# beecave-homelab/VibeVoice-ROCm

Measured on AMD Instinct MI355X. Metric: audio-sec/s, higher is better.
Workload: dtype bf16; 1 GPU; cfg2: VibeVoice-1.5B shapes, 1 speaker(s) x 203-frame voice prompt, 330-token prompt, 225 frames (30.0 s audio), CFG=2.0, 20 DPM-Solver++ steps, whole generate() incl. voice encode + prefill; global_batch=1, parallelism=replicas x1 (one dialogue per GPU), hipgraph=True

## Files before the change

### vibevoice_rocm_amd/build.py

```python
from __future__ import annotations

import hashlib
import os
import shutil
import subprocess
import sys

HERE = os.path.dirname(os.path.abspath(__file__))
ROOT = os.path.dirname(HERE)
SRC = [os.path.join(HERE, "csrc", f) for f in ("vv_kernels.hip", "vv_gemv_stream.hip", "vv_gemv_rows.hip", "vv_mfma_gemm.hip", "vv_block1d.hip", "vv_convffn.hip",
                                               "vv_fused.hip", "vv_attn_decode.hip", "vv_attn_prefill.hip", "vv_model.hip",
                                               "vv_nf4_import.hip")]
HDR = [os.path.join(ROOT, "include", "vv_hip.h"), os.path.join(HERE, "csrc", "vv_common.h")]
OUT = os.path.join(HERE, "libvv_hip.so")
OBJDIR = os.path.join(HERE, "csrc", "build")
STAMP = os.path.join(HERE, "libvv_hip.stamp")
FLAGS = ["--offload-arch=gfx950", "-O3", "-std=c++17", "-fPIC"]


def find_hipcc() -> str:
    for c in (os.environ.get("HIPCC"), shutil.which("hipcc"), "/opt/rocm/bin/hipcc"):
        if c and os.path.exists(c):
            return c
    raise RuntimeError("hipcc not found (ROCm toolchain required to build the MI355X kernels)")


def _flavour() -> str:
    return hashlib.sha256("\n".join([os.path.basename(s) for s in SRC] + FLAGS).encode()).hexdigest()[:16]


def _check_sources():
    missing = [p for p in SRC + HDR if not os.path.exists(p)]
    if missing:
        raise RuntimeError("missing kernel sources: " + ", ".join(os.path.relpath(p, ROOT) for p in missing))


def up_to_date() -> bool:
    if not os.path.exists(OUT):
        return False
    if not all(os.path.exists(p) for p in SRC + HDR):
        return True
    t = os.path.getmtime(OUT)
    if not all(os.path.getmtime(p) <= t for p in SRC + HDR):
        return False
    try:
        return open(STAMP).read().strip() == _flavour()
    except OSError:
        return False


def _obj(src: str) -> str:
    return os.path.join(OBJDIR, os.path.basename(src) + ".o")


def build(force: bool = False, verbose: bool = True, jobs: int = 6) -> str:
    if not force and up_to_date():
        return OUT
    _check_sources()
    os.makedirs(OBJDIR, exist_ok=True)
    flags = [*FLAGS, "-I" + os.path.join(ROOT, "include"), "-I" + os.path.join(HERE, "csrc")]
    hipcc = find_hipcc()
    hdr_t = max(os.path.getmtime(p) for p in HDR)
    todo = [s for s in SRC if force or not os.path.exists(_obj(s)) or os.path.getmtime(_obj(s)) < max(os.path.getmtime(s), hdr_t)]
    procs = []
    for s in todo:
        cmd = [hipcc, *flags, "-c", s, "-o", _obj(s)]
        if verbose:
            print(" ".join(cmd), flush=True)
        procs.append((s, subprocess.Popen(cmd)))
        while sum(p.poll() is None for _, p in procs) >= jobs:
            next(p for _, p in procs if p.poll() is None).wait()
    failed = [s for s, p in procs if p.wait() != 0]
    if failed:
        raise RuntimeError("hipcc failed for " + ", ".join(os.path.basename(f) for f in failed))
    cmd = [hipcc, "--offload-arch=gfx950", "-shared", "-fPIC", *[_obj(s) for s in SRC], "-o", OUT]
    if verbose:
        print(" ".join(cmd), flush=True)
    subprocess.run(cmd, check=True)
    with open(STAMP, "w") as f:
        f.write(_flavour() + "\n")
    return OUT


if __name__ == "__main__":
    build(force="--force" in sys.argv)
    print(OUT)
```

### vibevoice_rocm_amd/csrc/vv_common.h

```cpp
#ifndef VV_COMMON_H
#define VV_COMMON_H
#include <hip/hip_runtime.h>
#include <stdarg.h>
#include <stdint.h>
#include "vv_hip.h"

int vv_set_error(int code, const char* fmt, ...);

#define VV_CHECK_LAUNCH(name)                                                                    \
  do {                                                                                           \
    hipError_t e_ = hipGetLastError();                                                           \
    if (e_ != hipSuccess) return vv_set_error(VV_E_HIP, "%s: %s", name, hipGetErrorString(e_));  \
  } while (0)

#define VV_TRY(expr)            \
  do {                          \
    int rc_ = (expr);           \
    if (rc_) return rc_;        \
  } while (0)

int vv_launch_gemv_stream(const vv_lin_args& a, hipStream_t s);
int vv_launch_gemv_rows(const vv_lin_args& a, float* part, size_t part_floats, int* tickets, size_t n_tickets, hipStream_t s);
size_t vv_gemv_rows_part_floats(int n, int dual);
size_t vv_gemv_rows_tickets(int n);
int vv_gemv_rows_init();
void vv_gemv_rows_set(int on, int blocks, int pers);
int vv_linear_ws(const vv_lin_args* a, const void* f1, const void* f2, float* part, size_t part_floats, int* tickets, size_t n_tickets,
                 vv_stream_t stream, const vv_w8* q1 = nullptr, const vv_w8* q2 = nullptr);
int vv_launch_mfma_gemm(const vv_lin_args& a, hipStream_t s);
int vv_mfma_gemm_init();
int vv_launch_attn_decode(const float* qkv, int64_t ld_qkv, int R, int heads, const vv_kv* kv, int layer, const float2* rope, const int* lens, float* out,
                          int64_t ldo, float* part, int* tickets, int nsplit, int part_cap, hipStream_t s);
int vv_attn_decode_ws(const float* qkv, int64_t ld_qkv, int R, int heads, const vv_kv* kv, int layer, const float* rope_table, const int* lens, float* out,
                      int64_t ldo, float* part, int* tickets, int nsplit, int part_cap, vv_stream_t stream);
int vv_launch_attn_prefill(const float* qkv, int64_t ld_qkv, int R, int heads, const vv_kv* kv, int layer, const int* lens, const int* cache_rows,
                           float* out, int64_t ldo, hipStream_t s);
int vv_head_init_fused(const vv_head* h, const float* noise, float* Xs, float* Ms, float* h0, int64_t ldh, hipStream_t s);
bool vv_head_boundary_supported(const vv_head* h);
int vv_head_boundary_fused(const vv_head* h, const float* hrows, int64_t ldh, const float* shift, const float* scale, int64_t ld_mod, float cfg,
                           const vv_dpm_coef* k, float* Xs, float* Ms, float* h_out, int64_t ldh_out, float* latent_out, hipStream_t s);
int vv_head_boundary_batch(const vv_head* h, const float* hrows, int64_t ldh, const float* shift, const float* scale, int64_t ld_mod, float cfg,
                           const vv_dpm_coef* k, float* Xs, float* Ms, int64_t state_stride, float* h_out, int64_t ldh_out, float* latent_out,
                           int64_t latent_stride, int B, hipStream_t s,
                           const float* nx = nullptr, int64_t nx_stride = 0);
int vv_head_sde_proj_fused(const vv_head* h, const float* sde_noise, int64_t ld_sde, int n_steps, int B, float* NX, hipStream_t s);
int vv_fused_init();
int vv_head_pre_fused(const vv_head* h, const float* cond2, int64_t ld_cond, const float* temb, int n_steps, void* c_bf16, const float* noise,
                      float* Xs, float* Ms, float* h0, int64_t ldh, hipStream_t s);
int vv_launch_connector_pair(const vv_connector* ac, const vv_connector* sem, const float* latent, const float* semfeat, float* out, int64_t ldo, int rows_out,
                             float* ws, hipStream_t s);
int vv_head_modulations_fused(const vv_head* h, const void* c_bf16, int rows, float* const* mod, float* modf, hipStream_t s);
struct vv_conv_ctx_item { float* pad; float* state; int ctx, T, C; const float* dw_w; float* hs; int affine; float scale, bias; };
int vv_conv_ctx_batch(const vv_conv_ctx_item* items, int n, int scatter, hipStream_t s);
int vv_block1d_init();
int vv_launch_block1d(const vv_block& B, int wdt, const float* x, float* out, int T, int C, float eps, hipStream_t s);
void vv_block1d_set_fused(int on);
void vv_block1d_set_blocks(int b);
int vv_convffn_init();
int vv_launch_convffn(const vv_block& B, int wdt, const float* x, float* y, void* hidden, float* hist_new, float* out, int T, int C, float eps,
                      hipStream_t s);
void vv_convffn_set(int on);
int vv_launch_ffn_in_row(const vv_block& B, int wdt, const float* x, float* y, float* hidden, float* hist_new, int C, float eps, hipStream_t s);
void vv_convffn_set_t1(int on);
int vv_launch_ffn_in_row_hs(const vv_block& B, int wdt, const float* x, float* y, float* hidden, float* hist_new, int C, float eps, hipStream_t s);
void vv_convffn_set_t1hs(int on);
void vv_convffn_set_rows(int c, int rows);
void vv_convffn_set_c128(int on);
bool vv_convffn_prefers(int wdt, int T, int C);
int vv_launch_skinny(const vv_lin_args& a, hipStream_t s);
void vv_skinny_set(int on, int min_m, int max_m);
int vv_rmsnorm_rows(const float* x, int64_t ldx, const float* w, float eps, int rows, int n, float* out, int64_t ldo, hipStream_t s);

#ifdef __HIPCC__
__device__ __forceinline__ float vv_gelu_as(float v) {
  const float x = v * 0.70710678118654752440f, ax = fabsf(x);
  const float t = __builtin_amdgcn_rcpf(fmaf(0.3275911f, ax, 1.0f));
  const float poly = t * fmaf(t, fmaf(t, fmaf(t, fmaf(t, 1.061405429f, -1.453152027f), 1.421413741f), -0.284496736f), 0.254829592f);
  const float erf_abs = 1.0f - poly * __expf(-ax * ax);
  return 0.5f * v * (1.0f + copysignf(erf_abs, x));
}

__device__ __forceinline__ float vv_wave_sum(float v) {
#define VV_DPP_ADD(ctrl) v += __int_as_float(__builtin_amdgcn_update_dpp(0, __float_as_int(v), ctrl, 0xF, 0xF, true))
  VV_DPP_ADD(0xB1);
  VV_DPP_ADD(0x4E);
  VV_DPP_ADD(0x141);
  VV_DPP_ADD(0x140);
#undef VV_DPP_ADD
  const float r0 = __int_as_float(__builtin_amdgcn_readlane(__float_as_int(v), 0));
  const float r1 = __int_as_float(__builtin_amdgcn_readlane(__float_as_int(v), 16));
  const float r2 = __int_as_float(__builtin_amdgcn_readlane(__float_as_int(v), 32));
  const float r3 = __int_as_float(__builtin_amdgcn_readlane(__float_as_int(v), 48));
  return (r0 + r1) + (r2 + r3);
}
#endif

#endif
```

### vibevoice_rocm_amd/csrc/vv_gemv_stream.hip

```cpp
#include <hip/hip_runtime.h>
#include <stdint.h>

#include "vv_hip.h"
#include "vv_common.h"

namespace {

typedef unsigned short bf16_t;
typedef unsigned int u32x4 __attribute__((ext_vector_type(4)));

__device__ __forceinline__ float wsum(float v) { return vv_wave_sum(v); }
__device__ __forceinline__ float silu1(float v) { return v / (1.0f + expf(-v)); }
__device__ __forceinline__ float gelu1(float v) { return 0.5f * v * (1.0f + erff(v * 0.70710678118654752440f)); }

__device__ __forceinline__ void unpack8(const u32x4 v, float (&o)[8]) {
  o[0] = __uint_as_float(v.x << 16); o[1] = __uint_as_float(v.x & 0xffff0000u);
  o[2] = __uint_as_float(v.y << 16); o[3] = __uint_as_float(v.y & 0xffff0000u);
  o[4] = __uint_as_float(v.z << 16); o[5] = __uint_as_float(v.z & 0xffff0000u);
  o[6] = __uint_as_float(v.w << 16); o[7] = __uint_as_float(v.w & 0xffff0000u);
}

typedef unsigned int u32x2 __attribute__((ext_vector_type(2)));
typedef float f32x2 __attribute__((ext_vector_type(2)));
__device__ __forceinline__ void unpack8_f8(const u32x4 v, float (&o)[8]) {
// ... 450 lines not shown
    if (KSPLIT == 1) {
      if (lane < RW * M) {
        float v = acc[0][0], v2 = DUAL ? acc2[0][0] : 0.f;
#pragma unroll
        for (int r = 0; r < RW; ++r)
#pragma unroll
          for (int m = 0; m < M; ++m)
            if (lane == r * M + m) { v = acc[r][m]; if (DUAL) v2 = acc2[r][m]; }
        const int r = lane / M, m = lane - r * M;
        const int n = g * RW + r;
        if (n < N && m < mr) epi_pre(a, m, n, v, v2, eo_cur[0]);
      }
    } else {
      if (lane == 0) {
#pragma unroll
        for (int r = 0; r < RW; ++r)
#pragma unroll
          for (int m = 0; m < M; ++m) {
            part[parity][wave][(r * M + m) * 2] = acc[r][m];
            part[parity][wave][(r * M + m) * 2 + 1] = DUAL ? acc2[r][m] : 0.f;
          }
      }
      __syncthreads();
      if (tid < RW * M) {
        const int r = tid / M, m = tid - r * M;
        const int n = g * RW + r;
        if (n < N && m < mr) {
          float s = 0.f, s2 = 0.f;
#pragma unroll
          for (int w4 = 0; w4 < NW; ++w4) { s += part[parity][w4][tid * 2]; s2 += part[parity][w4][tid * 2 + 1]; }
          epi_pre(a, m, n, s, s2, eo_cur[0]);
        }
      }
      parity ^= 1;
    }
#pragma unroll
    for (int i = 0; i < NE; ++i) eo_cur[i] = eo_nxt[i];
#pragma unroll
    for (int r = 0; r < RW; ++r)
#pragma unroll
      for (int u = 0; u < KU; ++u) { cur[r][u] = nxt[r][u]; if (DUAL) cur2[r][u] = nxt2[r][u]; }
    g = gn;
    if (g + gstride < n_groups) { load_eo(eo_nxt, g + gstride); issue(nxt, nxt2, g + gstride); }
  }
}

int g_dual_rw = 1;

template <int M, bool DUAL, int KSPLIT, int KU, int RW>
void launch_rw(const vv_lin_args& a, hipStream_t s) {
  const int n_groups = (a.n + RW - 1) / RW;
  const int waves = (KSPLIT == 1 && g_waves_override >= 3 && g_waves_override <= 8) ? g_waves_override : 4;
  const int work = (KSPLIT == 1) ? (n_groups + waves - 1) / waves : n_groups;
  const int cap = (KSPLIT == 1) ? (DUAL ? (RW == 1 ? 512 : 448) : 512) : (a.k > 6144 ? g_long_cap : 1024);
  int blocks = work < cap ? work : cap;
  if (g_blocks_override > 0) blocks = g_blocks_override < work ? g_blocks_override : work;
  const int threads = KSPLIT == 1 ? 64 * waves : 64 * KSPLIT;
  if constexpr (RW == 4) {
    hipLaunchKernelGGL((gemv_stream_kernel<M, DUAL, KSPLIT, KU, RW, 2>), dim3(blocks), dim3(threads), 0, s, a, n_groups, g_opt);
    return;
  }
  if constexpr (M <= 2) {
    if (a.wdt == VV_FP8) {
      hipLaunchKernelGGL((gemv_stream_kernel<M, DUAL, KSPLIT, KU, RW, 1>), dim3(blocks), dim3(threads), 0, s, a, n_groups, g_opt);
      return;
    }
  }
  hipLaunchKernelGGL((gemv_stream_kernel<M, DUAL, KSPLIT, KU, RW, 0>), dim3(blocks), dim3(threads), 0, s, a, n_groups, g_opt);
}

int g_small_rw = 2;

template <int M, bool DUAL, int KSPLIT, int KU>
bool launch_one(const vv_lin_args& a, hipStream_t s) {
  if (a.wdt == VV_NF4) {
    if constexpr (M <= 2 && KSPLIT <= 8 && !(DUAL && KU > 4)) { launch_rw<M, DUAL, KSPLIT, KU, 4>(a, s); return true; }
    return false;
  }
  if (DUAL && g_dual_rw == 1) launch_rw<M, DUAL, KSPLIT, KU, 1>(a, s);
  else if (!DUAL && KSPLIT == 1 && a.n <= 4096 && g_small_rw == 1) launch_rw<M, DUAL, KSPLIT, KU, 1>(a, s);
  else launch_rw<M, DUAL, KSPLIT, KU, 2>(a, s);
  return true;
}

template <int M, bool DUAL, int KSPLIT>
bool launch_kus(const vv_lin_args& a, hipStream_t s, int ku) {
  switch (ku) {
    case 1: if constexpr (KSPLIT == 1) return launch_one<M, DUAL, KSPLIT, 1>(a, s); else return false;
    case 2: return launch_one<M, DUAL, KSPLIT, 2>(a, s);
    case 3: return launch_one<M, DUAL, KSPLIT, 3>(a, s);
    case 4: if constexpr (!DUAL || KSPLIT == 1) return launch_one<M, DUAL, KSPLIT, 4>(a, s); else return false;
    case 5: if constexpr (!DUAL || KSPLIT == 1) return launch_one<M, DUAL, KSPLIT, 5>(a, s); else return false;
  }
  return false;
}

template <int M, bool DUAL>
bool launch_ku(const vv_lin_args& a, hipStream_t s, int ksplit, int ku) {
  switch (ksplit) {
    case 1: return launch_kus<M, DUAL, 1>(a, s, ku);
    case 4: return launch_kus<M, DUAL, 4>(a, s, ku);
    case 8: return launch_kus<M, DUAL, 8>(a, s, ku);
    case 16: if constexpr (!DUAL) return launch_kus<M, false, 16>(a, s, ku); else return false;
  }
  return false;
}

bool launch_m8(const vv_lin_args& a, hipStream_t s, int ksplit, int ku) {
  if (ksplit == 1) {
    if (ku == 1) launch_rw<8, false, 1, 1, 1>(a, s); else launch_rw<8, false, 1, 2, 1>(a, s);
    return true;
  }
  switch (ksplit) {
    case 4: launch_rw<8, false, 4, 2, 2>(a, s); return true;
    case 8: launch_rw<8, false, 8, 2, 2>(a, s); return true;
  }
  return false;
}

}

void vv_gemv_stream_set_blocks(int b) { g_blocks_override = b; }
void vv_gemv_stream_set_waves(int w) { g_waves_override = w; }
void vv_gemv_stream_set_opt(int o) { g_opt = o; }
void vv_gemv_stream_set_long(int cap, int ku) { if (cap > 0) g_long_cap = cap; if (ku > 0) g_long_ku = ku; }
void vv_gemv_stream_set_dual_rw(int r) { g_dual_rw = r; }
void vv_gemv_stream_set_small_rw(int r) { g_small_rw = r; }

int vv_launch_gemv_stream(const vv_lin_args& a, hipStream_t s) {
  if ((a.wdt != VV_BF16 && a.wdt != VV_FP8 && a.wdt != VV_NF4) || a.m > 8 || a.k % 8) return 0;
  if (a.wdt == VV_NF4 && (a.m > 2 || a.k % 64 || !a.wscale || (a.w2 && !a.w2scale) || (uintptr_t)a.w % 16 || (a.w2 && (uintptr_t)a.w2 % 16) ||
                          (uintptr_t)a.wscale % 4 || (a.w2 && (uintptr_t)a.w2scale % 4) || (a.flags & VV_LIN_W_FRAG)))
    return 0;
  if (a.wdt == VV_FP8 && (a.m > 2 || !a.wscale || (a.w2 && !a.w2scale) || (uintptr_t)a.w % 8 || (a.w2 && (uintptr_t)a.w2 % 8))) return 0;
  if (a.m > 4) {
    if (a.w2 || a.wdt != VV_BF16) return 0;
    if ((uintptr_t)a.w % 16 || (uintptr_t)a.x % 16 || a.ldx % 4) return 0;
    if (a.norm_w && (uintptr_t)a.norm_w % 16) return 0;
    if (a.mod_scale && ((uintptr_t)a.mod_scale % 16 || (uintptr_t)a.mod_shift % 16 || a.ld_mod % 4)) return 0;
    const int units8 = (a.k + 511) / 512;
    int ks = 0, ku8 = 0;
    for (int w : {1, 4, 8}) {
      if ((units8 + w - 1) / w <= 2) { ks = w; ku8 = (units8 + w - 1) / w; break; }
    }
    if (!ks) return 0;
    if (ks > 1) ku8 = 2;
    return launch_m8(a, s, ks, ku8) ? 1 : 0;
  }
  if (a.wdt == VV_BF16 && ((uintptr_t)a.w % 16 || (a.w2 && (uintptr_t)a.w2 % 16))) return 0;
  if ((uintptr_t)a.x % 16) return 0;
  if (a.m > 1 && a.ldx % 4) return 0;
  if (a.norm_w && (uintptr_t)a.norm_w % 16) return 0;
  if (a.mod_scale && ((uintptr_t)a.mod_scale % 16 || (uintptr_t)a.mod_shift % 16 || a.ld_mod % 4)) return 0;
  const int units = (a.k + 511) / 512;
  const bool dual = a.w2 != nullptr;
  int ksplit = 1, ku = units;
  if (units > ((a.wdt == VV_NF4 && dual) ? 4 : 5)) {
    const int kumax = dual ? 3 : (units > 12 ? g_long_ku : 5);
    ksplit = 0;
    for (int w : {4, 8, 16}) {
      if ((units + w - 1) / w <= kumax) { ksplit = w; ku = (units + w - 1) / w; break; }
    }
    if (!ksplit) return 0;
    if (ku < 2) ku = 2;
  }
  if (a.wdt == VV_NF4 && ksplit > 8) return 0;
  bool ok;
  if (a.m == 1) ok = dual ? launch_ku<1, true>(a, s, ksplit, ku) : launch_ku<1, false>(a, s, ksplit, ku);
  else if (a.m == 2) ok = dual ? launch_ku<2, true>(a, s, ksplit, ku) : launch_ku<2, false>(a, s, ksplit, ku);
  else ok = dual ? launch_ku<4, true>(a, s, ksplit, ku) : launch_ku<4, false>(a, s, ksplit, ku);
  return ok ? 1 : 0;
}
```

### vibevoice_rocm_amd/csrc/vv_kernels.hip

```cpp
#include <hip/hip_runtime.h>
#include <hip/hip_bf16.h>
#include <stdint.h>
#include <stdio.h>
#include <string.h>
#include <math.h>

#include "vv_hip.h"
#include "vv_common.h"

static thread_local char g_err[512] = "";

int vv_set_error(int code, const char* fmt, ...) {
  va_list ap;
  va_start(ap, fmt);
  vsnprintf(g_err, sizeof(g_err), fmt, ap);
  va_end(ap);
  return code;
}

extern "C" const char* vv_last_error(void) { return g_err; }
extern "C" int vv_abi_version(void) { return 6; }
int vv_mixer_init();
extern "C" int vv_init(void) {
  VV_TRY(vv_mixer_init());
  VV_TRY(vv_mfma_gemm_init());
  VV_TRY(vv_block1d_init());
  VV_TRY(vv_convffn_init());
  VV_TRY(vv_gemv_rows_init());
  return vv_fused_init();
}
static float* g_rows_part = nullptr;
static int* g_rows_tk = nullptr;
static const size_t G_ROWS_PART_FLOATS = (size_t)4 << 20, G_ROWS_TICKETS = 4096;
static int rows_scratch(int on) {
  if (on && !g_rows_part) {
    if (hipMalloc(&g_rows_part, G_ROWS_PART_FLOATS * sizeof(float)) != hipSuccess || hipMalloc(&g_rows_tk, G_ROWS_TICKETS * sizeof(int)) != hipSuccess ||
        hipMemset(g_rows_tk, 0, G_ROWS_TICKETS * sizeof(int)) != hipSuccess)
      return vv_set_error(VV_E_HIP, "vv_tune: gemv_rows_scratch allocation failed");
  }
  if (!on && g_rows_part) { (void)hipFree(g_rows_part); (void)hipFree(g_rows_tk); g_rows_part = nullptr; g_rows_tk = nullptr; }
  return 0;
}
void vv_gemv_rows_set_dbg(int d);
void vv_gemv_rows_set_atomic(int on);
void vv_gemv_stream_set_blocks(int b);
void vv_gemv_stream_set_waves(int w);
void vv_gemv_stream_set_opt(int o);
void vv_gemv_stream_set_long(int cap, int ku);
void vv_gemv_stream_set_dual_rw(int r);
void vv_gemv_stream_set_small_rw(int r);
void vv_mfma_set_mt(int mt);
void vv_mfma_set_tiled_rows(int r);
void vv_mfma_set_tiled_bk128(int on);
void vv_mfma_set_tiled_small(int t);
void vv_mfma_set_tiled_dual_bk64(int on);
void vv_mfma_set_tiled_small_dual(int t);
void vv_mfma_set_tiled_small_k(int k);
void vv_mixer_set_rows(int on);
void vv_mfma_set_mt_prefill(int mt);
extern int g_attn_group;
void vv_attn_decode_set_gqa(int on);
void vv_attn_decode_set_gqa_keys(int k);
extern "C" int vv_tune(const char* key, int value) {
  if (key && !strcmp(key, "gemv_long_cap")) { vv_gemv_stream_set_long(value, 0); return 0; }
  if (key && !strcmp(key, "gemv_long_ku")) { vv_gemv_stream_set_long(0, value); return 0; }
  if (key && !strcmp(key, "gemv_blocks")) { vv_gemv_stream_set_blocks(value); return 0; }
  if (key && !strcmp(key, "gemv_waves")) { vv_gemv_stream_set_waves(value); return 0; }
  if (key && !strcmp(key, "gemv_rows")) { vv_gemv_rows_set(value, 0, -1); return 0; }
  if (key && !strcmp(key, "gemv_rows_blocks")) { vv_gemv_rows_set(-1, value, -1); return 0; }
  if (key && !strcmp(key, "gemv_rows_pers")) { vv_gemv_rows_set(-1, 0, value); return 0; }
  if (key && !strcmp(key, "gemv_rows_scratch")) return rows_scratch(value);
  if (key && !strcmp(key, "gemv_rows_dbg")) { vv_gemv_rows_set_dbg(value); return 0; }
  if (key && !strcmp(key, "gemv_rows_atomic")) { vv_gemv_rows_set_atomic(value); return 0; }
  if (key && !strcmp(key, "gemv_opt")) { vv_gemv_stream_set_opt(value); return 0; }
  if (key && !strcmp(key, "gemv_dual_rw")) { vv_gemv_stream_set_dual_rw(value); return 0; }
  if (key && !strcmp(key, "gemv_small_rw")) { vv_gemv_stream_set_small_rw(value); return 0; }
  if (key && !strcmp(key, "mixer_rows")) { vv_mixer_set_rows(value); return 0; }
  if (key && !strcmp(key, "block1d_fused")) { vv_block1d_set_fused(value); return 0; }
  if (key && !strcmp(key, "block1d_blocks")) { vv_block1d_set_blocks(value); return 0; }
  if (key && !strcmp(key, "convffn")) { vv_convffn_set(value); return 0; }
  if (key && !strcmp(key, "convffn_t1")) { vv_convffn_set_t1(value); return 0; }
  if (key && !strcmp(key, "convffn_t1hs")) { vv_convffn_set_t1hs(value); return 0; }
  if (key && !strcmp(key, "convffn_rows512")) { vv_convffn_set_rows(512, value); return 0; }
  if (key && !strcmp(key, "convffn_rows256")) { vv_convffn_set_rows(256, value); return 0; }
  if (key && !strcmp(key, "convffn_rows128")) { vv_convffn_set_rows(128, value); return 0; }
  if (key && !strcmp(key, "convffn_c128")) { vv_convffn_set_c128(value); return 0; }
  if (key && !strcmp(key, "skinny")) { vv_skinny_set(value, 0, 0); return 0; }
  if (key && !strcmp(key, "skinny_min_m")) { vv_skinny_set(1, value, 0); return 0; }
  if (key && !strcmp(key, "skinny_max_m")) { vv_skinny_set(1, 0, value); return 0; }
  if (key && !strcmp(key, "mfma_tiled_bk128")) { vv_mfma_set_tiled_bk128(value); return 0; }
  if (key && !strcmp(key, "attn_group")) { g_attn_group = value; return 0; }
  if (key && !strcmp(key, "attn_gqa")) { vv_attn_decode_set_gqa(value); return 0; }
  if (key && !strcmp(key, "attn_gqa_keys")) { vv_attn_decode_set_gqa_keys(value); return 0; }
  if (key && !strcmp(key, "mfma_tiled_small_k")) { vv_mfma_set_tiled_small_k(value); return 0; }
  if (key && !strcmp(key, "mfma_tiled_dual_bk64")) { vv_mfma_set_tiled_dual_bk64(value); return 0; }
  if (key && !strcmp(key, "mfma_tiled_small_dual")) { vv_mfma_set_tiled_small_dual(value); return 0; }
  if (key && !strcmp(key, "mfma_tiled_small")) { vv_mfma_set_tiled_small(value); return 0; }
  if (key && !strcmp(key, "mfma_tiled_rows")) { vv_mfma_set_tiled_rows(value); return 0; }
  if (key && !strcmp(key, "mfma_mt")) { vv_mfma_set_mt(value); return 0; }
  if (key && !strcmp(key, "mfma_mt_prefill")) { vv_mfma_set_mt_prefill(value); return 0; }
  return vv_set_error(VV_E_ARG, "vv_tune: unknown key");
}

typedef unsigned short bf16_t;

__device__ __forceinline__ float bf2f(unsigned int u16) { return __uint_as_float(u16 << 16); }
__device__ __forceinline__ float wave_sum(float v) {
#pragma unroll
  for (int o = 32; o > 0; o >>= 1) v += __shfl_xor(v, o);
  return v;
}
__device__ __forceinline__ float wave_sum_dpp(float v) { return vv_wave_sum(v); }
__device__ __forceinline__ float silu_f(float v) { return v / (1.0f + expf(-v)); }
__device__ __forceinline__ float gelu_f(float v) { return 0.5f * v * (1.0f + erff(v * 0.70710678118654752440f)); }

template <typename WT> struct WL;
template <> struct WL<float> {
  static __device__ __forceinline__ void load8(const float* p, float (&o)[8]) {
    const float4 a = *reinterpret_cast<const float4*>(p);
    const float4 b = *reinterpret_cast<const float4*>(p + 4);
    o[0] = a.x; o[1] = a.y; o[2] = a.z; o[3] = a.w; o[4] = b.x; o[5] = b.y; o[6] = b.z; o[7] = b.w;
  }
  static __device__ __forceinline__ void load4(const float* p, float (&o)[4]) {
    const float4 a = *reinterpret_cast<const float4*>(p);
    o[0] = a.x; o[1] = a.y; o[2] = a.z; o[3] = a.w;
  }
  static __device__ __forceinline__ float load1(const float* p) { return *p; }
};
template <> struct WL<bf16_t> {
  static __device__ __forceinline__ void load8(const bf16_t* p, float (&o)[8]) {
    const uint4 v = *reinterpret_cast<const uint4*>(p);
    o[0] = __uint_as_float(v.x << 16); o[1] = __uint_as_float(v.x & 0xffff0000u);
    o[2] = __uint_as_float(v.y << 16); o[3] = __uint_as_float(v.y & 0xffff0000u);
    o[4] = __uint_as_float(v.z << 16); o[5] = __uint_as_float(v.z & 0xffff0000u);
    o[6] = __uint_as_float(v.w << 16); o[7] = __uint_as_float(v.w & 0xffff0000u);
  }
  static __device__ __forceinline__ void load4(const bf16_t* p, float (&o)[4]) {
    const uint2 v = *reinterpret_cast<const uint2*>(p);
    o[0] = __uint_as_float(v.x << 16); o[1] = __uint_as_float(v.x & 0xffff0000u);
    o[2] = __uint_as_float(v.y << 16); o[3] = __uint_as_float(v.y & 0xffff0000u);
  }
  static __device__ __forceinline__ float load1(const bf16_t* p) { return bf2f(*p); }
};

__device__ __forceinline__ void lin_epilogue(const vv_lin_args& a, int m, int n, float v, float v2) {
  if (a.bias) v += a.bias[n];
  if (a.act == VV_ACT_GELU) v = gelu_f(v);
  else if (a.act == VV_ACT_SWIGLU) v = silu_f(v) * v2;
  if (a.gate) v *= a.gate_ld ? a.gate[(int64_t)m * a.gate_ld + n] : a.gate[n];
  if (a.res) v += a.res[(int64_t)m * a.ldres + n];
  a.out[(int64_t)m * a.ldo + n] = v;
}

#define GEMV_THREADS 256

template <int M>
__device__ __forceinline__ void row_stats(const vv_lin_args& a, float* red, float (&rstd)[M]) {
  const int tid = threadIdx.x, lane = tid & 63, wave = tid >> 6;
  float ss[M];
#pragma unroll
  for (int m = 0; m < M; ++m) {
    const float* xr = a.x + (int64_t)m * a.ldx;
    float s = 0.f;
    for (int k = tid; k < a.k; k += GEMV_THREADS) { const float v = xr[k]; s += v * v; }
    ss[m] = wave_sum(s);
  }
  if (lane == 0) {
#pragma unroll
    for (int m = 0; m < M; ++m) red[wave * M + m] = ss[m];
  }
  __syncthreads();
#pragma unroll
  for (int m = 0; m < M; ++m) {
    const float t = red[m] + red[M + m] + red[2 * M + m] + red[3 * M + m];
    rstd[m] = rsqrtf(t / (float)a.k + a.eps);
  }
  __syncthreads();
}

template <int M>
__device__ __forceinline__ void stage_chunk(const vv_lin_args& a, float* xs, int kc0, int kc, int kcp, const float (&rstd)[M]) {
  for (int idx = threadIdx.x; idx < M * kcp; idx += GEMV_THREADS) {
    const int m = idx / kcp, kk = idx - m * kcp;
    float v = 0.f;
    if (kk < kc) {
      const int k = kc0 + kk;
      v = a.x[(int64_t)m * a.ldx + k];
      if (a.pro == VV_PRO_RMSNORM) {
        v *= rstd[m];
        if (a.norm_w) v *= a.norm_w[k];
        if (a.mod_scale) v = v * (1.0f + a.mod_scale[(int64_t)m * a.ld_mod + k]) + a.mod_shift[(int64_t)m * a.ld_mod + k];
      } else if (a.pro == VV_PRO_SILU) {
        v = silu_f(v);
      }
    }
    xs[idx] = v;
  }
}

template <typename WT, int M, bool DUAL, int KSPLIT, int RW>
__global__ __launch_bounds__(GEMV_THREADS) void gemv_kernel(const vv_lin_args a, const int KC) {
  extern __shared__ __attribute__((aligned(16))) float smem[];
  float* red = smem;
  float* xs = smem + 64 * 4;
  const int tid = threadIdx.x, lane = tid & 63, wave = tid >> 6;
  const int K = a.k, N = a.n;
  const WT* __restrict__ W = reinterpret_cast<const WT*>(a.w);
  const WT* __restrict__ W2 = reinterpret_cast<const WT*>(a.w2);

  float rstd[M];
#pragma unroll
  for (int m = 0; m < M; ++m) rstd[m] = 1.f;
  if (a.pro == VV_PRO_RMSNORM) row_stats<M>(a, red, rstd);

  const int row0 = (KSPLIT == 1 ? (blockIdx.x * 4 + wave) : blockIdx.x) * RW;
  float acc[RW][M], acc2[DUAL ? RW : 1][M];
#pragma unroll
  for (int r = 0; r < RW; ++r)
#pragma unroll
    for (int m = 0; m < M; ++m) { acc[r][m] = 0.f; if (DUAL) acc2[r][m] = 0.f; }

  for (int kc0 = 0; kc0 < K; kc0 += KC) {
    const int kc = min(KC, K - kc0);
    const int kcp = (kc + 7) & ~7;
    if (kc0 > 0) __syncthreads();
    stage_chunk<M>(a, xs, kc0, kc, kcp, rstd);
    __syncthreads();
    const int kstart = (KSPLIT == 1 ? lane : (wave * 64 + lane)) * 8;
    const int kstep = (KSPLIT == 1 ? 64 : 256) * 8;
// ... 1477 lines not shown
```

Baseline: 38.34 audio-sec/s.

## Add shape-specialized fused GEMV kernels for hot M=2 bf16 linears

Adds a new source file with compile-time-specialized GEMV kernels for the six hottest M=2 bf16 shapes (CFG pair): the diffusion-head and LLM gate/up with fused RMSNorm+modulation+SwiGLU, the down projections with gate/residual epilogues, and QKV/O. All weights are issued as up-front register loads, with nontemporal loads for the streaming LLM weights. The stream GEMV dispatcher tries these first. This is meant to cut per-call overhead and improve bandwidth use over the generic path, at the cost of register pressure and more code to maintain.

```diff
diff --git a/vibevoice_rocm_amd/build.py b/vibevoice_rocm_amd/build.py
--- a/vibevoice_rocm_amd/build.py
+++ b/vibevoice_rocm_amd/build.py
@@ -8,7 +8,7 @@
 
 HERE = os.path.dirname(os.path.abspath(__file__))
 ROOT = os.path.dirname(HERE)
-SRC = [os.path.join(HERE, "csrc", f) for f in ("vv_kernels.hip", "vv_gemv_stream.hip", "vv_gemv_rows.hip", "vv_mfma_gemm.hip", "vv_block1d.hip", "vv_convffn.hip",
+SRC = [os.path.join(HERE, "csrc", f) for f in ("vv_kernels.hip", "vv_gemv_stream.hip", "vv_gemv_hot.hip", "vv_gemv_rows.hip", "vv_mfma_gemm.hip", "vv_block1d.hip", "vv_convffn.hip",
                                                "vv_fused.hip", "vv_attn_decode.hip", "vv_attn_prefill.hip", "vv_model.hip",
                                                "vv_nf4_import.hip")]
 HDR = [os.path.join(ROOT, "include", "vv_hip.h"), os.path.join(HERE, "csrc", "vv_common.h")]
diff --git a/vibevoice_rocm_amd/csrc/vv_common.h b/vibevoice_rocm_amd/csrc/vv_common.h
--- a/vibevoice_rocm_amd/csrc/vv_common.h
+++ b/vibevoice_rocm_amd/csrc/vv_common.h
@@ -20,6 +20,10 @@
   } while (0)
 
 int vv_launch_gemv_stream(const vv_lin_args& a, hipStream_t s);
+struct vv_gemv_hot_shape { const char* name; int m, n, k, dual, pro, mod, bias, gate, res, act, flags; };
+extern "C" int vv_gemv_hot_shapes(vv_gemv_hot_shape* out, int cap);
+int vv_launch_gemv_hot(const vv_lin_args& a, hipStream_t s);
+void vv_gemv_hot_set(int mask);
 int vv_launch_gemv_rows(const vv_lin_args& a, float* part, size_t part_floats, int* tickets, size_t n_tickets, hipStream_t s);
 size_t vv_gemv_rows_part_floats(int n, int dual);
 size_t vv_gemv_rows_tickets(int n);
diff --git a/vibevoice_rocm_amd/csrc/vv_gemv_hot.hip b/vibevoice_rocm_amd/csrc/vv_gemv_hot.hip
--- /dev/null
+++ b/vibevoice_rocm_amd/csrc/vv_gemv_hot.hip
@@ -0,0 +1,401 @@
+#include <hip/hip_runtime.h>
+#include <stdint.h>
+
+#include "vv_hip.h"
+#include "vv_common.h"
+
+namespace {
+
+typedef unsigned short bf16_t;
+typedef unsigned int u32x4 __attribute__((ext_vector_type(4)));
+typedef float vf2 __attribute__((ext_vector_type(2)));
+
+__device__ __forceinline__ float silu1(float v) { return v / (1.0f + expf(-v)); }
+
+__device__ __forceinline__ void unpack8(const u32x4 v, float (&o)[8]) {
+  o[0] = __uint_as_float(v.x << 16); o[1] = __uint_as_float(v.x & 0xffff0000u);
+  o[2] = __uint_as_float(v.y << 16); o[3] = __uint_as_float(v.y & 0xffff0000u);
+  o[4] = __uint_as_float(v.z << 16); o[5] = __uint_as_float(v.z & 0xffff0000u);
+  o[6] = __uint_as_float(v.w << 16); o[7] = __uint_as_float(v.w & 0xffff0000u);
+}
+
+template <bool NT>
+__device__ __forceinline__ u32x4 ldw(const bf16_t* p) {
+  const u32x4* q = reinterpret_cast<const u32x4*>(p);
+  if constexpr (NT) return __builtin_nontemporal_load(q);
+  else return *q;
+}
+
+__device__ __forceinline__ void fma_unit(const u32x4 wv, const float (&x0)[8], const float (&x1)[8], vf2& p0, vf2& p1) {
+  float w[8];
+  unpack8(wv, w);
+#pragma unroll
+  for (int j = 0; j < 8; j += 2) p0 = __builtin_elementwise_fma(vf2{w[j], w[j + 1]}, vf2{x0[j], x0[j + 1]}, p0);
+#pragma unroll
+  for (int j = 0; j < 8; j += 2) p1 = __builtin_elementwise_fma(vf2{w[j], w[j + 1]}, vf2{x1[j], x1[j + 1]}, p1);
+}
+
+__device__ __forceinline__ float vv_hot_gate_res(float v, float g, float r) {
+#pragma clang fp contract(off)
+  const float t = v * g;
+  return t + r;
+}
+
+#define VV_FENCE4(v) asm volatile("" : "+v"((v).x), "+v"((v).y), "+v"((v).z), "+v"((v).w))
+
+template <int N, bool MOD, bool NT>
+__global__ __launch_bounds__(256, 2) void hot_dual_kernel(const vv_lin_args a) {
+  constexpr int K = 1536, KU = 3, M = 2, T = 256, NCH = 2, NCHUNKS = K / 4;
+  constexpr int WAVES = 512 * 4, G = (N + WAVES - 1) / WAVES;
+  constexpr bool RAGGED = (N % WAVES) != 0;
+  __shared__ float red[4 * M];
+  __shared__ __attribute__((aligned(16))) float xs[M * KU * 512];
+  const int tid = threadIdx.x, lane = tid & 63;
+  const int wave = __builtin_amdgcn_readfirstlane(tid >> 6);
+  const int gw = wave * 512 + (int)blockIdx.x;
+  const bf16_t* __restrict__ W = reinterpret_cast<const bf16_t*>(a.w);
+  const bf16_t* __restrict__ W2 = reinterpret_cast<const bf16_t*>(a.w2);
+
+  float4 xv[M][NCH], nv[NCH], sv[M][NCH], cv[M][NCH];
+#pragma unroll
+  for (int c = 0; c < NCH; ++c) {
+    const int ch = tid + c * T;
+    const int kk = ch < NCHUNKS ? ch * 4 : 0;
+#pragma unroll
+    for (int m = 0; m < M; ++m) xv[m][c] = *reinterpret_cast<const float4*>(a.x + (int64_t)m * a.ldx + kk);
+    nv[c] = *reinterpret_cast<const float4*>(a.norm_w + kk);
+    if constexpr (MOD) {
+#pragma unroll
+      for (int m = 0; m < M; ++m) {
+        const int64_t mo = (int64_t)m * a.ld_mod + kk;
+        sv[m][c] = *reinterpret_cast<const float4*>(a.mod_shift + mo);
+        cv[m][c] = *reinterpret_cast<const float4*>(a.mod_scale + mo);
+      }
+    }
+  }
+  u32x4 wq[G][KU], wq2[G][KU];
+#pragma unroll
+  for (int i = 0; i < G; ++i) {
+    const int n = gw + i * WAVES;
+    const bool live = !RAGGED || i < G - 1 || n < N;
+    const int off = live ? n * K + lane * 8 : 0;
+#pragma unroll
+    for (int u = 0; u < KU; ++u) {
+      wq[i][u] = ldw<NT>(W + off + (live ? u * 512 : 0));
+      wq2[i][u] = ldw<NT>(W2 + off + (live ? u * 512 : 0));
+    }
+  }
+  __builtin_amdgcn_sched_barrier(0);
+#pragma unroll
+  for (int c = 0; c < NCH; ++c) {
+#pragma unroll
+    for (int m = 0; m < M; ++m) VV_FENCE4(xv[m][c]);
+    VV_FENCE4(nv[c]);
+    if constexpr (MOD) {
+#pragma unroll
+      for (int m = 0; m < M; ++m) { VV_FENCE4(sv[m][c]); VV_FENCE4(cv[m][c]); }
+    }
+  }
+
+  float ss[M];
+#pragma unroll
+  for (int m = 0; m < M; ++m) {
+    float s1 = 0.f;
+#pragma unroll
+    for (int c = 0; c < NCH; ++c) {
+      const float4 v = xv[m][c];
+      s1 += (tid + c * T < NCHUNKS) ? (v.x * v.x + v.y * v.y) + (v.z * v.z + v.w * v.w) : 0.f;
+    }
+    ss[m] = vv_wave_sum(s1);
+  }
+  if (lane == 0) {
+#pragma unroll
+    for (int m = 0; m < M; ++m) red[wave * M + m] = ss[m];
+  }
+  __syncthreads();
+#pragma unroll
+  for (int m = 0; m < M; ++m) {
+    float tot = 0.f;
+#pragma unroll
+    for (int w4 = 0; w4 < 4; ++w4) tot += red[w4 * M + m];
+    const float rstd = rsqrtf(tot / (float)a.k + a.eps);
+#pragma unroll
+    for (int c = 0; c < NCH; ++c) {
+      const int ch = tid + c * T;
+      float4 v = xv[m][c];
+      v.x *= rstd; v.y *= rstd; v.z *= rstd; v.w *= rstd;
+      v.x *= nv[c].x; v.y *= nv[c].y; v.z *= nv[c].z; v.w *= nv[c].w;
+      if constexpr (MOD) {
+        v.x = v.x * (1.0f + cv[m][c].x) + sv[m][c].x; v.y = v.y * (1.0f + cv[m][c].y) + sv[m][c].y;
+        v.z = v.z * (1.0f + cv[m][c].z) + sv[m][c].z; v.w = v.w * (1.0f + cv[m][c].w) + sv[m][c].w;
+      }
+      if (ch < NCHUNKS) *reinterpret_cast<float4*>(&xs[(m * KU * 128 + ch) * 4]) = v;
+    }
+  }
+  __syncthreads();
+  float xr[M][KU][8];
+#pragma unroll
+  for (int m = 0; m < M; ++m)
+#pragma unroll
+    for (int u = 0; u < KU; ++u) {
+      const float4 p = *reinterpret_cast<const float4*>(&xs[m * KU * 512 + u * 512 + lane * 8]);
+      const float4 q = *reinterpret_cast<const float4*>(&xs[m * KU * 512 + u * 512 + lane * 8 + 4]);
+      xr[m][u][0] = p.x; xr[m][u][1] = p.y; xr[m][u][2] = p.z; xr[m][u][3] = p.w;
+      xr[m][u][4] = q.x; xr[m][u][5] = q.y; xr[m][u][6] = q.z; xr[m][u][7] = q.w;
+    }
+
+#pragma unroll
+  for (int i = 0; i < G; ++i) {
+    const int n = gw + i * WAVES;
+    if (RAGGED && i == G - 1 && n >= N) break;
+    vf2 p[M] = {vf2{0.f, 0.f}, vf2{0.f, 0.f}}, p2[M] = {vf2{0.f, 0.f}, vf2{0.f, 0.f}};
+#pragma unroll
+    for (int u = 0; u < KU; ++u) {
+      fma_unit(wq[i][u], xr[0][u], xr[1][u], p[0], p[1]);
+      fma_unit(wq2[i][u], xr[0][u], xr[1][u], p2[0], p2[1]);
+    }
+    float acc[M], acc2[M];
+#pragma unroll
+    for (int m = 0; m < M; ++m) {
+      acc[m] = vv_wave_sum(p[m].x + p[m].y);
+      acc2[m] = vv_wave_sum(p2[m].x + p2[m].y);
+    }
+    if (lane < M) {
+      const float v = lane == 0 ? acc[0] : acc[1], v2 = lane == 0 ? acc2[0] : acc2[1];
+      a.out[(int64_t)lane * a.ldo + n] = silu1(v) * v2;
+    }
+  }
+}
+
+template <int N, int WPB, bool RMS, bool NT>
+__global__ __launch_bounds__(64 * WPB) void hot_rows_kernel(const vv_lin_args a) {
+  constexpr int K = 1536, KU = 3, M = 2, RW = 2;
+  static_assert(N % (RW * WPB) == 0, "every wave of the grid owns one whole row pair");
+  const int tid = threadIdx.x, lane = tid & 63;
+  const int wave = __builtin_amdgcn_readfirstlane(tid >> 6);
+  const int g = (int)blockIdx.x * WPB + wave;
+  const bf16_t* __restrict__ W = reinterpret_cast<const bf16_t*>(a.w);
+
+  float4 xa[M][KU], xb[M][KU], na[KU], nb[KU];
+#pragma unroll
+  for (int m = 0; m < M; ++m) {
+    const float* xrow = a.x + (int64_t)m * a.ldx + lane * 8;
+#pragma unroll
+    for (int u = 0; u < KU; ++u) {
+      xa[m][u] = *reinterpret_cast<const float4*>(xrow + u * 512);
+      xb[m][u] = *reinterpret_cast<const float4*>(xrow + u * 512 + 4);
+    }
+  }
+  if constexpr (RMS) {
+#pragma unroll
+    for (int u = 0; u < KU; ++u) {
+      na[u] = *reinterpret_cast<const float4*>(a.norm_w + u * 512 + lane * 8);
+      nb[u] = *reinterpret_cast<const float4*>(a.norm_w + u * 512 + lane * 8 + 4);
+    }
+  }
+  const int eo_id = lane < RW * M ? lane : 0;
+  const int eo_r = eo_id >> 1, eo_m = eo_id & 1;
+  const int eo_n = g * RW + eo_r;
+  float eo;
+  if constexpr (RMS) eo = a.bias[eo_n];
+  else eo = a.res[(int64_t)eo_m * a.ldres + eo_n];
+  u32x4 wq[RW][KU];
+#pragma unroll
+  for (int r = 0; r < RW; ++r)
+#pragma unroll
+    for (int u = 0; u < KU; ++u) wq[r][u] = ldw<NT>(W + (g * RW + r) * K + u * 512 + lane * 8);
+  __builtin_amdgcn_sched_barrier(0);
+#pragma unroll
+  for (int u = 0; u < KU; ++u) {
+#pragma unroll
+    for (int m = 0; m < M; ++m) { VV_FENCE4(xa[m][u]); VV_FENCE4(xb[m][u]); }
+    if constexpr (RMS) { VV_FENCE4(na[u]); VV_FENCE4(nb[u]); }
+  }
+
+  float xr[M][KU][8];
+  float ss[M];
+#pragma unroll
+  for (int m = 0; m < M; ++m) {
+    ss[m] = 0.f;
+#pragma unroll
+    for (int u = 0; u < KU; ++u) {
+      xr[m][u][0] = xa[m][u].x; xr[m][u][1] = xa[m][u].y; xr[m][u][2] = xa[m][u].z; xr[m][u][3] = xa[m][u].w;
+      xr[m][u][4] = xb[m][u].x; xr[m][u][5] = xb[m][u].y; xr[m][u][6] = xb[m][u].z; xr[m][u][7] = xb[m][u].w;
+      if constexpr (RMS) {
+#pragma unroll
+        for (int j = 0; j < 8; ++j) ss[m] = fmaf(xr[m][u][j], xr[m][u][j], ss[m]);
+      }
+    }
+  }
+  if constexpr (RMS) {
+#pragma unroll
+    for (int m = 0; m < M; ++m) ss[m] = vv_wave_sum(ss[m]);
+#pragma unroll
+    for (int m = 0; m < M; ++m) {
+      const float rstd = rsqrtf(ss[m] / (float)a.k + a.eps);
+#pragma unroll
+      for (int u = 0; u < KU; ++u) {
+        const float nw[8] = {na[u].x, na[u].y, na[u].z, na[u].w, nb[u].x, nb[u].y, nb[u].z, nb[u].w};
+#pragma unroll
+        for (int j = 0; j < 8; ++j) {
+          float v = xr[m][u][j] * rstd;
+          v *= nw[j];
+          xr[m][u][j] = v;
+        }
+      }
+    }
+  }
+
+  vf2 p[RW][M];
+#pragma unroll
+  for (int r = 0; r < RW; ++r) {
+    p[r][0] = vf2{0.f, 0.f}; p[r][1] = vf2{0.f, 0.f};
+#pragma unroll
+    for (int u = 0; u < KU; ++u) fma_unit(wq[r][u], xr[0][u], xr[1][u], p[r][0], p[r][1]);
+  }
+  float acc[RW][M];
+#pragma unroll
+  for (int r = 0; r < RW; ++r)
+#pragma unroll
+    for (int m = 0; m < M; ++m) acc[r][m] = vv_wave_sum(p[r][m].x + p[r][m].y);
+  if (lane < RW * M) {
+    const float v0 = (lane & 1) ? acc[0][1] : acc[0][0], v1 = (lane & 1) ? acc[1][1] : acc[1][0];
+    float v = (lane & 2) ? v1 : v0;
+    v += eo;
+    a.out[(int64_t)eo_m * a.ldo + eo_n] = v;
+  }
+}
+
+template <int N, int K, int R, bool GATE, bool NT>
+__global__ __launch_bounds__(256) void hot_down_kernel(const vv_lin_args a) {
+  constexpr int M = 2, NW = 4, UNITS = (K + 511) / 512, KU = (UNITS + NW - 1) / NW;
+  static_assert(N % R == 0 && R * M <= 64, "whole row sets; the epilogue threads are the first R * M of the block");
+  __shared__ float part[NW][R * M];
+  const int tid = threadIdx.x, lane = tid & 63;
+  const int wave = __builtin_amdgcn_readfirstlane(tid >> 6);
+  const int n0 = (int)blockIdx.x * R;
+  const bf16_t* __restrict__ W = reinterpret_cast<const bf16_t*>(a.w);
+
+  int koff[KU];
+  bool kval[KU];
+#pragma unroll
+  for (int u = 0; u < KU; ++u) {
+    koff[u] = (wave + NW * u) * 512 + lane * 8;
+    kval[u] = koff[u] < K;
+    if (!kval[u]) koff[u] = 0;
+  }
+  float4 xa[M][KU], xb[M][KU];
+#pragma unroll
+  for (int m = 0; m < M; ++m) {
+    const float* xrow = a.x + (int64_t)m * a.ldx;
+#pragma unroll
+    for (int u = 0; u < KU; ++u) {
+      xa[m][u] = *reinterpret_cast<const float4*>(xrow + koff[u]);
+      xb[m][u] = *reinterpret_cast<const float4*>(xrow + koff[u] + 4);
+    }
+  }
+  const int eo_id = tid < R * M ? tid : 0;
+  const int eo_r = eo_id >> 1, eo_m = eo_id & 1;
+  const int eo_n = n0 + eo_r;
+  float eg = 1.f;
+  if constexpr (GATE) eg = a.gate[(int64_t)eo_m * a.gate_ld + eo_n];
+  const float er = a.res[(int64_t)eo_m * a.ldres + eo_n];
+  u32x4 wq[R][KU];
+#pragma unroll
+  for (int r = 0; r < R; ++r)
+#pragma unroll
+    for (int u = 0; u < KU; ++u) wq[r][u] = ldw<NT>(W + (n0 + r) * K + koff[u]);
+  __builtin_amdgcn_sched_barrier(0);
+#pragma unroll
+  for (int u = 0; u < KU; ++u)
+#pragma unroll
+    for (int m = 0; m < M; ++m) { VV_FENCE4(xa[m][u]); VV_FENCE4(xb[m][u]); }
+
+  float xr[M][KU][8];
+#pragma unroll
+  for (int m = 0; m < M; ++m)
+#pragma unroll
+    for (int u = 0; u < KU; ++u) {
+      const bool kv = kval[u];
+      xr[m][u][0] = kv ? xa[m][u].x : 0.f; xr[m][u][1] = kv ? xa[m][u].y : 0.f; xr[m][u][2] = kv ? xa[m][u].z : 0.f; xr[m][u][3] = kv ? xa[m][u].w : 0.f;
+      xr[m][u][4] = kv ? xb[m][u].x : 0.f; xr[m][u][5] = kv ? xb[m][u].y : 0.f; xr[m][u][6] = kv ? xb[m][u].z : 0.f; xr[m][u][7] = kv ? xb[m][u].w : 0.f;
+    }
+
+  float acc[R][M];
+#pragma unroll
+  for (int r = 0; r < R; ++r) {
+    vf2 p0 = vf2{0.f, 0.f}, p1 = vf2{0.f, 0.f};
+#pragma unroll
+    for (int u = 0; u < KU; ++u) fma_unit(wq[r][u], xr[0][u], xr[1][u], p0, p1);
+    acc[r][0] = vv_wave_sum(p0.x + p0.y);
+    acc[r][1] = vv_wave_sum(p1.x + p1.y);
+  }
+  if (lane == 0) {
+#pragma unroll
+    for (int r = 0; r < R; ++r) { part[wave][r * M] = acc[r][0]; part[wave][r * M + 1] = acc[r][1]; }
+  }
+  __syncthreads();
+  if (tid < R * M) {
+    float s = 0.f;
+#pragma unroll
+    for (int w4 = 0; w4 < NW; ++w4) s += part[w4][tid];
+    float v = s;
+    if constexpr (GATE) v = vv_hot_gate_res(v, eg, er);
+    else v += er;
+    a.out[(int64_t)eo_m * a.ldo + eo_n] = v;
+  }
+}
+
+#undef VV_FENCE4
+
+constexpr int N_HOT = 6;
+const vv_gemv_hot_shape g_table[N_HOT] = {
+    {"head.gate_up", 2, 4608, 1536, 1, VV_PRO_RMSNORM, 1, 0, 0, 0, VV_ACT_SWIGLU, VV_LIN_W_REUSED},
+    {"head.down",    2, 1536, 4608, 0, VV_PRO_NONE,    0, 0, 1, 1, VV_ACT_NONE,   VV_LIN_W_REUSED},
+    {"llm.gate_up",  2, 8960, 1536, 1, VV_PRO_RMSNORM, 0, 0, 0, 0, VV_ACT_SWIGLU, 0},
+    {"llm.down",     2, 1536, 8960, 0, VV_PRO_NONE,    0, 0, 0, 1, VV_ACT_NONE,   0},
+    {"llm.qkv",      2, 2048, 1536, 0, VV_PRO_RMSNORM, 0, 1, 0, 0, VV_ACT_NONE,   0},
+    {"llm.o",        2, 1536, 1536, 0, VV_PRO_NONE,    0, 0, 0, 1, VV_ACT_NONE,   0},
+};
+
+constexpr int HOT_DEFAULT = 0x3f;
+int g_hot = HOT_DEFAULT;
+
+bool matches(const vv_gemv_hot_shape& e, const vv_lin_args& a) {
+  return a.m == e.m && a.n == e.n && a.k == e.k && a.wdt == VV_BF16 && (a.w2 != nullptr) == (e.dual != 0) && a.pro == e.pro &&
+         (a.pro != VV_PRO_RMSNORM || a.norm_w != nullptr) && (a.mod_scale != nullptr) == (e.mod != 0) && (!e.mod || a.mod_shift != nullptr) &&
+         (a.bias != nullptr) == (e.bias != 0) && (a.gate != nullptr) == (e.gate != 0) && (!e.gate || a.gate_ld != 0) &&
+         (a.res != nullptr) == (e.res != 0) && a.act == e.act && a.flags == e.flags;
+}
+
+}
+
+void vv_gemv_hot_set(int mask) { g_hot = mask < 0 ? HOT_DEFAULT : mask; }
+
+extern "C" int vv_gemv_hot_shapes(vv_gemv_hot_shape* out, int cap) {
+  for (int i = 0; i < N_HOT && i < cap; ++i) out[i] = g_table[i];
+  return N_HOT;
+}
+
+int vv_launch_gemv_hot(const vv_lin_args& a, hipStream_t s) {
+  if (!(g_hot & ((1 << N_HOT) - 1)) || a.m != 2 || a.wdt != VV_BF16) return 0;
+  int id = -1;
+  for (int i = 0; i < N_HOT; ++i)
+    if ((g_hot >> i & 1) && matches(g_table[i], a)) { id = i; break; }
+  const bool r3 = (g_hot & 256) != 0;
+  switch (id) {
+    case 0: hipLaunchKernelGGL((hot_dual_kernel<4608, true, false>), dim3(512), dim3(256), 0, s, a); return 1;
+    case 1:
+      if (r3) hipLaunchKernelGGL((hot_down_kernel<1536, 4608, 3, true, false>), dim3(512), dim3(256), 0, s, a);
+      else hipLaunchKernelGGL((hot_down_kernel<1536, 4608, 6, true, false>), dim3(256), dim3(256), 0, s, a);
+      return 1;
+    case 2: hipLaunchKernelGGL((hot_dual_kernel<8960, false, true>), dim3(512), dim3(256), 0, s, a); return 1;
+    case 3:
+      if (r3) hipLaunchKernelGGL((hot_down_kernel<1536, 8960, 3, false, true>), dim3(512), dim3(256), 0, s, a);
+      else hipLaunchKernelGGL((hot_down_kernel<1536, 8960, 6, false, true>), dim3(256), dim3(256), 0, s, a);
+      return 1;
+    case 4: hipLaunchKernelGGL((hot_rows_kernel<2048, 4, true, true>), dim3(256), dim3(256), 0, s, a); return 1;
+    case 5: hipLaunchKernelGGL((hot_rows_kernel<1536, 3, false, true>), dim3(256), dim3(192), 0, s, a); return 1;
+  }
+  return 0;
+}
diff --git a/vibevoice_rocm_amd/csrc/vv_gemv_stream.hip b/vibevoice_rocm_amd/csrc/vv_gemv_stream.hip
--- a/vibevoice_rocm_amd/csrc/vv_gemv_stream.hip
+++ b/vibevoice_rocm_amd/csrc/vv_gemv_stream.hip
@@ -626,6 +626,7 @@
   if (a.m > 1 && a.ldx % 4) return 0;
   if (a.norm_w && (uintptr_t)a.norm_w % 16) return 0;
   if (a.mod_scale && ((uintptr_t)a.mod_scale % 16 || (uintptr_t)a.mod_shift % 16 || a.ld_mod % 4)) return 0;
+  if (a.m == 2 && a.wdt == VV_BF16 && vv_launch_gemv_hot(a, s)) return 1;
   const int units = (a.k + 511) / 512;
   const bool dual = a.w2 != nullptr;
   int ksplit = 1, ku = units;
diff --git a/vibevoice_rocm_amd/csrc/vv_kernels.hip b/vibevoice_rocm_amd/csrc/vv_kernels.hip
--- a/vibevoice_rocm_amd/csrc/vv_kernels.hip
+++ b/vibevoice_rocm_amd/csrc/vv_kernels.hip
@@ -75,6 +75,7 @@
   if (key && !strcmp(key, "gemv_opt")) { vv_gemv_stream_set_opt(value); return 0; }
   if (key && !strcmp(key, "gemv_dual_rw")) { vv_gemv_stream_set_dual_rw(value); return 0; }
   if (key && !strcmp(key, "gemv_small_rw")) { vv_gemv_stream_set_small_rw(value); return 0; }
+  if (key && !strcmp(key, "gemv_hot")) { vv_gemv_hot_set(value); return 0; }
   if (key && !strcmp(key, "mixer_rows")) { vv_mixer_set_rows(value); return 0; }
   if (key && !strcmp(key, "block1d_fused")) { vv_block1d_set_fused(value); return 0; }
   if (key && !strcmp(key, "block1d_blocks")) { vv_block1d_set_blocks(value); return 0; }
```

New measurement: 42.29 audio-sec/s, median of 6. 10.3% higher.
